# mlee03/FRE-NCtools

Hardware: AMD Instinct MI355X
Metric: exchange-cells/s (higher is better)
Workload: dtype f64; 1 GPU; C384 cubed sphere (6 tiles) -> 1440x720 lat-lon, conservative_order2: exchange-grid search + centroid pass + CSR build per step; nxgrid=4160000, parallelism=1 latitude band(s) of the target, one per GPU, world_size=1

## Files before the change

fre-nctools_amd/_lib.py:

```python
import ctypes as C
import os

_HERE = os.path.dirname(os.path.abspath(__file__))
_LIB = None


class FregridHipError(RuntimeError):
    def __init__(self, code, msg):
        super().__init__(f"libfregrid_hip error {code}: {msg}")
        self.code = code


def lib_path():
    return os.environ.get("FREGRID_HIP_LIB") or os.path.join(_HERE, "libfregrid_hip.so")


EXPORTS = [
    "get_maxxgrid", "get_grid_area", "create_xgrid_2dx2d_order1", "create_xgrid_2dx2d_order2", "conserve_interp",
    "clip_2dx2d", "poly_area", "poly_ctrlon", "poly_ctrlat", "fix_lon", "pimod",
    "fg_clip_2dx2d_batch", "fg_poly_op_batch",
    "get_maxxgrid_", "get_grid_area_", "create_xgrid_2dx2d_order1_", "create_xgrid_2dx2d_order2_",
    "fg_last_error", "fg_device_count", "fg_plan_create", "fg_plan_create_dev", "fg_plan_create_empty",
    "fg_plan_destroy", "fg_plan_set_stream", "fg_pool_release", "fg_plan_nxgrid", "fg_plan_ncells_in",
    "fg_plan_cell_sums_dev", "fg_plan_copy_cell_sums", "fg_plan_accumulate_cell_sums", "fg_plan_accumulate_cell_sums_async", "fg_dev_gather_f64", "fg_dev_scatter_f64", "fg_plan_finalize", "fg_plan_get_xgrid", "fg_plan_get_polygons", "fg_plan_create_polylist", "fg_plan_get_cell_struct",
# ... 1 lines not shown
    "fg_plan_mono_minmax_dev", "fg_plan_mono_copy_minmax", "fg_plan_mono_end",
    "fg_plan_create_great_circle", "fg_plan_create_great_circle_dev", "fg_latlon2xyz", "create_xgrid_great_circle",
    "create_xgrid_great_circle_", "get_grid_great_circle_area", "get_grid_great_circle_area_", "clip_2dx2d_great_circle",
    "great_circle_area", "fg_gc_clip_batch", "conserve_interp_great_circle", "fg_sincos_batch",
    "create_xgrid_1dx2d_order1", "create_xgrid_1dx2d_order2", "create_xgrid_2dx1d_order1", "create_xgrid_2dx1d_order2",
    "create_xgrid_1dx2d_order1_", "create_xgrid_1dx2d_order2_", "create_xgrid_2dx1d_order1_", "create_xgrid_2dx1d_order2_",
    "clip", "box_ctrlat", "box_ctrlon", "get_grid_area_no_adjust", "get_grid_area_no_adjust_", "fg_plan_stream", "fg_plan_sync",
    "fg_c2l_create", "fg_c2l_destroy", "fg_c2l_ncells", "fg_c2l_halo_size", "fg_c2l_set_stream", "fg_c2l_sync",
    "fg_c2l_get_centres", "fg_c2l_fill_halo", "fg_c2l_gradient", "fg_c2l_gradient_records", "fg_c2l_records", "fg_c2l_records_levels", "fg_c2l_grid_info", "fg_find_contacts", "fg_halo_map",
    "fg_gnomonic_ed_grid", "fg_tripolar_corners", "fg_remap_write", "fg_remap_write_interp", "fg_remap_read_size", "fg_remap_read", "fg_remap_last_error",
    "fg_plan_trim", "fg_plan_ncells_out", "fg_plan_order", "fg_plan_device", "fg_dev_alloc", "fg_dev_free", "fg_dev_upload", "fg_dev_download",
    "fg_nc_open", "fg_nc_create", "fg_nc_def_dim", "fg_nc_def_var", "fg_nc_put_att_text", "fg_nc_put_att_double", "fg_nc_enddef",
    "fg_nc_inq_ndims", "fg_nc_inq_nvars", "fg_nc_inq_numrecs", "fg_nc_inq_dimid", "fg_nc_inq_dim", "fg_nc_inq_varid", "fg_nc_inq_var",
    "fg_nc_get_att_double", "fg_nc_get_att_text", "fg_nc_get_vara", "fg_nc_get_vara_double", "fg_nc_put_vara", "fg_nc_put_vara_double",
    "fg_nc_close", "fg_nc_last_error", "fg_dev_widen", "fg_dev_narrow", "fg_sweep_create", "fg_sweep_run", "fg_sweep_run_levels", "fg_sweep_destroy", "fg_host_alloc", "fg_host_free",
    "fg_plan_stats", "fg_set_search_mode", "fg_set_search_cull", "fg_set_search_finalize", "fg_set_search_rect", "fg_set_search_wide_cap", "fg_set_search_frame", "fg_set_apply_xcd", "fg_set_apply_vec", "fg_set_apply_ep", "fg_set_gc_split", "fg_set_profiling", "fg_plan_phase_ms", "fg_gnomonic_ed_corners", "fg_latlon_corners",
    "fg_bilin_create", "fg_bilin_create_from_weights", "fg_bilin_destroy", "fg_bilin_get_index_weight", "fg_bilin_npoints_fine",
    "fg_bilin_nlon_fine", "fg_bilin_nlat_fine", "fg_bilin_nlon", "fg_bilin_nlat", "fg_bilin_ncells", "fg_bilin_set_stream",
    "fg_bilin_sync", "fg_bilin_apply_scalar", "fg_bilin_apply_vector", "fg_bilin_remap_write", "fg_bilin_remap_read",
    "fg_unit_vect_latlon", "fg_bilin_fine_grid", "fg_bilin_ambiguous_ties",
    "fg_extrap_create", "fg_extrap_destroy", "fg_extrap_set_stream", "fg_extrap_stream", "fg_extrap_run_dev", "fg_extrap_run",
    "fg_extrap_last_syncs", "fg_extrap_get_coef", "fg_extrap_coef_host", "fg_set_extrap_batch", "fg_set_extrap_coef",
    "fg_setup_vertical_interp", "fg_dev_vertical_interp",
    "fg_dev_latlon2xyz", "fg_plan_create_great_circle_lonlat", "fg_plan_create_great_circle_lonlat_dev",
    "fg_runoff_create", "fg_runoff_create_from_xgrid", "fg_runoff_destroy", "fg_runoff_nxgrid", "fg_runoff_get_xgrid",
    "fg_runoff_get_maps", "fg_runoff_get_xyz", "fg_runoff_search_stats", "fg_runoff_phase_ms", "fg_runoff_stream", "fg_runoff_apply", "fg_runoff_apply_dev",
    "fg_nearest_unmasked", "fg_set_runoff_prune", "fg_runoff_tile",
    "fg_rland_create", "fg_rland_destroy", "fg_rland_stream", "fg_rland_search", "fg_rland_search_sface", "fg_rland_stats",
    "fg_rland_phase_ms", "fg_set_rland_prune", "fg_rland_tile",
    "fg_river_create", "fg_river_destroy", "fg_river_stream", "fg_river_run", "fg_river_get", "fg_river_get_max_suba",
    "fg_river_stats", "fg_river_phase_ms", "fg_set_river_prune", "fg_river_qsort_index",
# ... 478 lines not shown
```

fre-nctools_amd/csrc/plan.hip:

```cpp
#include <hip/hip_runtime.h>
#include <math.h>
#include <stdio.h>
#include <stdlib.h>
#include <string.h>
#include <algorithm>
#include <map>
#include <mutex>
#include <string>
#include <type_traits>
#include <vector>
#include "fg_host.h"
#include "plan_internal.h"
#include "xgrid_device.h"

static thread_local std::string g_err;
extern "C" const char *fg_last_error(void) { return g_err.c_str(); }
void fg_set_last_error(const char *msg) { g_err = msg ? msg : ""; }

extern "C" int fg_device_count(void)
{
  int n = 0;
  hipError_t e = hipGetDeviceCount(&n);
  if (e != hipSuccess) { fg_fail(FG_ERR_HIP, "hipGetDeviceCount: %s", hipGetErrorString(e)); return FG_ERR_HIP; }
  return n;
}

namespace {
struct Pool {
  std::mutex mu;
  std::map<std::pair<int, size_t>, std::vector<void *>> free_;
  std::map<void *, std::pair<int, size_t>> live_;
  static size_t klass(size_t n)
  {
    size_t c = 256;
    while (c < n) c += (c < (1u << 20) ? c : (c >> 2));
    return c;
  }
  static void *poison(void *p, size_t c)
  {
    static const bool on = getenv("FREGRID_HIP_POISON") && atoi(getenv("FREGRID_HIP_POISON")) != 0;
    if (on && p) { (void)hipMemset(p, 0x7f, c); (void)hipDeviceSynchronize(); }
    return p;
  }
  void *get(int dev, size_t n) { return poison(get_raw(dev, n), klass(n ? n : 1)); }
  void *get_raw(int dev, size_t n)
  {
    if (n == 0) n = 1;
    size_t c = klass(n);
    {
      std::lock_guard<std::mutex> lk(mu);
      auto it = free_.find({dev, c});
      if (it != free_.end() && !it->second.empty()) {
        void *p = it->second.back(); it->second.pop_back();
        live_[p] = {dev, c};
        return p;
      }
    }
    void *p = nullptr;
    if (hipMalloc(&p, c) != hipSuccess) {
      release_all();
      if (hipMalloc(&p, c) != hipSuccess) return nullptr;
    }
    std::lock_guard<std::mutex> lk(mu);
    live_[p] = {dev, c};
    return p;
  }
  void put(void *p)
  {
    if (!p) return;
    std::lock_guard<std::mutex> lk(mu);
    auto it = live_.find(p);
    if (it == live_.end()) return;
    free_[it->second].push_back(p);
    live_.erase(it);
  }
  void release_all()
  {
    std::lock_guard<std::mutex> lk(mu);
    for (auto &kv : free_) for (void *p : kv.second) (void)hipFree(p);
    free_.clear();
  }
};
Pool g_pool;
}

extern "C" void fg_pool_release(void) { g_pool.release_all(); }

extern "C" void *fg_dev_alloc(size_t bytes, int device)
{
  if (hipSetDevice(device) != hipSuccess) { fg_fail(FG_ERR_HIP, "fg_dev_alloc: no such HIP device %d", device); return nullptr; }
  void *p = g_pool.get(device, bytes);
  if (!p) fg_fail(FG_ERR_HIP, "fg_dev_alloc: out of device memory (%zu bytes)", bytes);
  return p;
}
extern "C" void fg_dev_free(void *p) { g_pool.put(p); }
extern "C" int fg_dev_upload(void *dst_dev, const void *src_host, size_t bytes)
{
// ... 136 lines not shown
    }
    cv_work.notify_all();
    std::unique_lock<std::mutex> lk(mu);
    cv_done.wait(lk, [&] { return active == 0; });
    jobs = nullptr;
    return failed.load() == 0;
  }
};
XferPool &xfer_pool() { static XferPool *p = new XferPool(); return *p; }
}

static int g_profiling = 0;
extern "C" void fg_set_profiling(int on) { g_profiling = on ? 1 : 0; }
enum { PH_CELL_STRUCT = 0, PH_BINS, PH_CANDIDATES, PH_CLIP_QUAD, PH_CLIP_GENERAL, PH_COMPACT, PH_ROWS,
       PH_SEARCH_TOTAL, PH_FINALIZE, PH_APPLY, PH_COUNT };
struct HandleCache {
  std::mutex mu;
  std::map<int, std::vector<hipStream_t>> streams;
  std::map<int, std::vector<hipEvent_t>> events;
  static int current_device() { int d = 0; (void)hipGetDevice(&d); return d; }
  hipStream_t get_stream(int dev)
  {
    {
      std::lock_guard<std::mutex> lk(mu);
      auto &v = streams[dev];
      if (!v.empty()) { hipStream_t s = v.back(); v.pop_back(); return s; }
    }
    hipStream_t s = nullptr;
    if (hipStreamCreateWithFlags(&s, hipStreamNonBlocking) != hipSuccess) return nullptr;
    return s;
  }
  void put_stream(int dev, hipStream_t s)
  {
    if (!s) return;
    std::lock_guard<std::mutex> lk(mu);
    streams[dev].push_back(s);
  }
  hipEvent_t get_event()
  {
    {
      std::lock_guard<std::mutex> lk(mu);
      auto &v = events[current_device()];
      if (!v.empty()) { hipEvent_t e = v.back(); v.pop_back(); return e; }
    }
    hipEvent_t e = nullptr;
    (void)hipEventCreate(&e);
    return e;
  }
  void put_event(hipEvent_t e)
  {
    if (!e) return;
    std::lock_guard<std::mutex> lk(mu);
    events[current_device()].push_back(e);
  }
  std::map<int, std::vector<hipEvent_t>> sync_events;
  hipEvent_t get_sync_event()
  {
    {
      std::lock_guard<std::mutex> lk(mu);
      auto &v = sync_events[current_device()];
      if (!v.empty()) { hipEvent_t e = v.back(); v.pop_back(); return e; }
    }
    hipEvent_t e = nullptr;
    (void)hipEventCreateWithFlags(&e, hipEventDisableTiming);
    return e;
  }
  void put_sync_event(hipEvent_t e)
  {
    if (!e) return;
    std::lock_guard<std::mutex> lk(mu);
    sync_events[current_device()].push_back(e);
  }
};
static HandleCache g_handles;

struct PhaseTimer {
  bool on = false;
  hipStream_t st = nullptr;
  std::vector<std::pair<int, std::pair<hipEvent_t, hipEvent_t>>> spans;
  hipEvent_t open_ev = nullptr; int open_ph = -1;
  void start(bool enable, hipStream_t s) { on = enable; st = s; }
  void begin(int ph)
  {
    if (!on) return;
    open_ev = g_handles.get_event(); (void)hipEventRecord(open_ev, st); open_ph = ph;
  }
  void end()
  {
    if (!on || open_ph < 0) return;
// ... 47 lines not shown
  FgSrcRec *cen = nullptr;
  FgCsr csr{};
  int *src_idx_f = nullptr;
  double *row_sum = nullptr, *red_partial = nullptr, *red_result = nullptr;
  long row_sum_cap = 0;
  double *il_f = nullptr, *il_out = nullptr, *il_rs = nullptr;
  double *il_m = nullptr;
  unsigned char *lv_bits = nullptr;
  long stats[FG_NSTATS] = {0};
  long search_d2h = 0;
  double *mono_x = nullptr, *mono_b = nullptr;
  int *xerr = nullptr;
  bool mono_open = false;
  unsigned *ll_err = nullptr;

  template <typename T> T *alloc(size_t count)
  {
    void *p = g_pool.get(device, count * sizeof(T));
    if (p) owned.push_back(p);
    return (T *)p;
  }
  void release(void *p)
  {
    if (!p) return;
    for (size_t k = 0; k < owned.size(); k++) if (owned[k] == p) { owned.erase(owned.begin() + k); break; }
    g_pool.put(p);
  }
  void drop_search(size_t keep)
  {
    while (owned.size() > keep) { g_pool.put(owned.back()); owned.pop_back(); }
    tiles_dev = nullptr; mask_dev = nullptr; S = FgCells{}; D = FgCells{};
    x_src = x_dst = nullptr; x_area = x_c1 = x_c2 = nullptr; xoff = nullptr;
    perm = nullptr; csr.row_ptr = nullptr; csr.e1 = nullptr; csr.e2 = nullptr; cen = nullptr; src_idx_f = nullptr; sums = nullptr;
    have_geom = false; rect = false; rect_tab = FgRect{};
  }
};

static int g_wide_cap = -1;
extern "C" void fg_set_search_wide_cap(int n) { g_wide_cap = n < 0 ? -1 : n; }
static bool alloc_cells(fg_plan *pl, FgCells *c, size_t n, bool compact = false)
{
// ... 29 lines not shown
    foff += (order == 2) ? (long)(nx_in[m] + 2) * (ny_in[m] + 2) : (long)nx_in[m] * ny_in[m];
  }
  if (off > 2000000000L || (long)nx_out * ny_out > 2000000000L) { delete pl; return fg_fail(FG_ERR_ARG, "grid too large for 32-bit cell indices"); }
  pl->nsrc = (int)off; pl->f_stride = foff;
  pl->nx_out = nx_out; pl->ny_out = ny_out; pl->ndst = nx_out * ny_out;
  pl->stream = g_handles.get_stream(device);
  if (!pl->stream) { delete pl; return fg_fail(FG_ERR_HIP, "hipStreamCreate failed"); }
  *out = pl;
  return 0;
}

extern "C" void fg_plan_destroy(fg_plan *pl)
{
  if (!pl) return;
  (void)hipSetDevice(pl->device);
  if (pl->stream || !pl->own_stream) (void)hipStreamSynchronize(pl->stream);
  if (pl->stream && pl->own_stream) g_handles.put_stream(pl->device, pl->stream);
  if (pl->stream_b) { (void)hipStreamSynchronize(pl->stream_b); g_handles.put_stream(pl->device, pl->stream_b); }
  { float junk[PH_COUNT] = {0}; pl->apply_pt.collect(junk); }
  for (void *p : pl->owned) g_pool.put(p);
  delete pl;
}

static void choose_bins(const fg_plan *pl, double mean_dlat, double mean_dlon, FgBins *b)
{
  const double PI = 3.14159265358979323846;
  double h = 1.25 * mean_dlat, w = 1.25 * mean_dlon;
  int nblat = (h > 0) ? (int)ceil(PI / h) : 1;
  int nblon = (w > 0) ? (int)ceil(2.0 * PI / w) : 1;
  if (nblat < 1) nblat = 1; if (nblat > 8192) nblat = 8192;
  if (nblon < 1) nblon = 1; if (nblon > 16384) nblon = 16384;
  (void)pl;
  b->nblat = nblat; b->nblon = nblon;
  b->inv_wlat = nblat / PI;
  b->inv_wlon = nblon / (2.0 * PI);
}

static FgCounters *pinned_counters()
{
  static thread_local FgCounters *h = nullptr;
  if (!h) { if (hipHostMalloc((void **)&h, sizeof(FgCounters), hipHostMallocDefault) != hipSuccess) h = nullptr; }
  return h;
}

struct GcXyz { const double *x, *y, *z; };
struct BoxMode { FgBox box; const double *mask_quad; int no_adjust; };
struct SearchIn {
  const double *const *lon_in = nullptr, *const *lat_in = nullptr, *const *mask_in = nullptr;
  const double *lon_out = nullptr, *lat_out = nullptr;
  const GcXyz *gc_in = nullptr, *gc_out = nullptr;
  const BoxMode *boxm = nullptr;
  double mean_dlat = 0, mean_dlon = 0;
  int rect_hint = 1;
};
struct SearchOpts { bool exact, cull, finalize, rect, dst_frame; int gc_split; bool profile; };
static const char *gc_clip_error(int code)
{
  switch (code) {
    case 3: return "firstIntersect is not in the grid1List";
    case 4: return " not found the next intersection ";
    case 5: return "not return back to the first intersection";
    case 6: return "After clipping, nintersect should be 0";
    case 7: return "inserAfter: point (x,y,z) is not found in the list";
    case 8: return "Error from create_xgrid.c: temp is not in list1";
    default: return "clip_2dx2d_great_circle: more intersections than two convex quadrilaterals can have (list capacity)";
  }
}

static int g_search_cull = 0;
static int g_search_finalize = 0;
// ... 248 lines not shown
  io.dc = dc; io.xcap = nx_alloc;
  if (early_rows)
    fgd_exclusive_scan2(nacc, nsrc, pl->xoff, lb_comp, &tickets[2], &dc->xtot, row_cnt, ndst, pl->csr.row_ptr, lb_rows, &tickets[1], &dc->rows_total, dc->err, st);
  else
    fgd_exclusive_scan1(nacc, nsrc, pl->xoff, lb_comp, &tickets[2], &dc->xtot, dc->err, st);
  fgd_compact(order, nsrc, ps, io, st);
  pt.end();
  if (!early_rows) {
    pt.begin(PH_ROWS);
    fgd_exclusive_scan1(row_cnt, ndst, pl->csr.row_ptr, lb_rows, &tickets[1], &dc->rows_total, dc->err, st);
    fgd_csr_fill_pos(nx_alloc, &dc->xtot, pl->x_src, pl->x_dst, pl->csr.row_ptr, x_rowpos, pl->perm, st);
    pt.end();
  }
  ptot.end();
  const bool fuse = opt.finalize && early_rows && !pl->polys.npoly;
  int *fused_tmp = nullptr;
  if (fuse) {
    pt.begin(PH_FINALIZE);
    if (order == 2) {
      pl->cen = pl->alloc<FgSrcRec>((size_t)nsrc + 1);
      if (!pl->cen) return fg_fail(FG_ERR_HIP, "out of device memory");
      fgd_centroids(nsrc, pl->S, pl->sums, pl->cen, st);
      pl->csr.e2 = pl->alloc<FgCsrEntry2>(nx_alloc + 1);
    } else pl->csr.e1 = pl->alloc<FgCsrEntry1>(nx_alloc + 1);
    if (!pl->csr.e1 && !pl->csr.e2) return fg_fail(FG_ERR_HIP, "out of device memory");
    int *sg_tmp = pl->alloc<int>(3 * (size_t)(nx_alloc + 1));
    fgd_csr_sortgather(order, ndst, (long)nsrc + ndst, pl->perm, pl->x_area, pl->x_c1, pl->x_c2, pl->src_idx_f,
                       order == 2 ? pl->cen : nullptr, pl->csr, st, sg_tmp, nx_alloc + 1);
    fused_tmp = sg_tmp;
    pt.end();
  }
  FGCHK(hipMemcpyAsync(hc, dc, sizeof(FgCounters), hipMemcpyDeviceToHost, st));
  FGCHK(hipStreamSynchronize(st));
  pt.collect(pl->phase_ms); ptot.collect(pl->phase_ms);
  FGCHK(hipGetLastError());
  if (rect && hc->rect_bad) { caps->rect = false; return FG_RETRY; }
  if (rect && (hc->err[0] & G_ERRBIT_WIDECAP)) { caps->rect = false; return FG_RETRY; }
  if (hc->total[0] > nentries) { caps->entries = hc->total[0]; return FG_RETRY; }
  if (hc->total[0] > 2000000000ull) return fg_fail(FG_ERR_ARG, "bin table too large");
  if (hc->total[3] > (unsigned long long)ps.regcap) {
    if (hc->total[3] > 2000000000ull / (unsigned long long)ps.nreg) return fg_fail(FG_ERR_CAPACITY, "candidate pair list exceeds 2^31 entries");
    caps->regcap = (int)((hc->total[3] + FG_REG_ALIGN - 1) / FG_REG_ALIGN * FG_REG_ALIGN);
    return FG_RETRY;
  }
  if (hc->err[2] & G_ERRBIT_LL2X) return fg_fail(FG_ERR_ARG, "latlon2xyz: a grid corner is not finite, or its latitude (|lat| >= 2.4262) or longitude "
                                                          "(|lon| > 1024) lies outside the range of the device trig (radians expected)");
  if (hc->err[0] & 8u) return fg_fail(FG_ERR_ARG, "a grid corner latitude lies outside [-pi/2, pi/2] (radians expected)");
  if (hc->err[0] & 1u) return fg_fail(FG_ERR_MAXV, "create_xgrid.c: n2_in is greater than MAX_V");
// ... 5 lines not shown
  if (hc->err[0] & G_ERRBIT_GC_CLIP) return fg_fail(FG_ERR_GEOM, "%s", gc_clip_error((int)hc->err[1]));
  if (hc->err[0] & G_ERRBIT_LOOKBACK) return fg_fail(FG_ERR_HIP, "single-pass scan: a tile waited too long for its predecessor");
  pl->nx = (long)hc->xtot;
  pl->stats[FG_STAT_PAIRS] = (long)hc->total[1];
  pl->stats[FG_STAT_NONEMPTY] = (long)(hc->xtot + hc->stats[FG_STAT_BELOW]);
  pl->stats[FG_STAT_NXGRID] = pl->nx;
  pl->stats[FG_STAT_BORDERLINE] = (long)hc->stats[FG_STAT_BORDERLINE];
  pl->stats[FG_STAT_BINS] = nbins;
  pl->stats[FG_STAT_BIN_ENTRIES] = (long)hc->total[0];
  pl->stats[FG_STAT_DEFERRED] = hc->defer_cnt + hc->gc_list2_cnt;
  pl->stats[FG_STAT_HEAVY] = hc->heavy_cnt;
  pl->stats[FG_STAT_RARE] = hc->rare_cnt;
  pl->stats[FG_STAT_BELOW] = (long)hc->stats[FG_STAT_BELOW];

  pl->rect_tab.bad = nullptr;
  blk.release();
  pl->rows_built = true;
  pl->searched = true;
  if (fuse) {
    pl->release(pl->perm); pl->perm = nullptr; pl->release(fused_tmp);
    if (!pl->red_partial) { pl->red_partial = pl->alloc<double>(1024); pl->red_result = pl->alloc<double>(260); }
    if (!pl->red_partial || !pl->red_result) return fg_fail(FG_ERR_HIP, "out of device memory");
    pl->dist_pending = (order == 2);
    pl->finalized = true; pl->fused = true;
  }
  return pl->nx;
}

static int g_search_exact = 0;
extern "C" void fg_set_search_mode(int exact) { g_search_exact = exact; }
extern "C" void fg_set_search_cull(int on) { g_search_cull = on ? 1 : 0; }
extern "C" void fg_set_search_finalize(int on) { g_search_finalize = on ? 1 : 0; }
static long plan_search(fg_plan *pl, const SearchIn &in)
{
  static const bool env_exact = getenv("FREGRID_HIP_EXACT_SEARCH") && atoi(getenv("FREGRID_HIP_EXACT_SEARCH")) != 0;
  const SearchOpts opt{.exact = g_search_exact || env_exact, .cull = g_search_cull != 0, .finalize = g_search_finalize != 0,
                       .rect = g_search_rect != 0, .dst_frame = (tl_dst_frame >= 0 ? tl_dst_frame : g_dst_frame) != 0, .gc_split = g_gc_split, .profile = g_profiling != 0};
  const long big = std::max((long)pl->nsrc, (long)pl->ndst);
  if (big > (1L << 28)) return fg_fail(FG_ERR_CAPACITY, "grid of %ld cells: more than 2^28 cells per search are not supported", big);
  SearchCaps caps;
  caps.entries = opt.exact ? 0ull : 3ull * (unsigned long long)pl->ndst + 4096ull;
  const unsigned long long cap_pairs = std::min<unsigned long long>(8ull * (unsigned long long)big + 65536ull, 2000000000ull);
  caps.nreg = (int)std::max(1L, std::min((long)FG_NREG, ((long)pl->nsrc + 1023) / 1024));
  caps.regcap = opt.exact ? 0 : (int)((cap_pairs / caps.nreg + FG_REG_ALIGN - 1) / FG_REG_ALIGN * FG_REG_ALIGN);
  caps.rect = opt.rect && in.rect_hint && !in.gc_in && !in.boxm && pl->nx_out <= 8192 && pl->nx_out >= 2;
  const size_t keep = pl->owned.size();
  long rc = FG_RETRY;
  int attempts = 0;
  for (; attempts < 4 && rc == FG_RETRY; attempts++) {
    if (attempts) {
      (void)hipStreamSynchronize(pl->stream);
      pl->drop_search(keep);
    }
    rc = plan_search_core(pl, in, opt, &caps);
  }
  if (rc == FG_RETRY) return fg_fail(FG_ERR_CAPACITY, "exchange-grid search: capacities did not settle");
  if (rc >= 0) pl->stats[FG_STAT_EXACT] = (attempts > 1) ? 1 : 0;
  pl->search_d2h = (long)attempts * (long)sizeof(FgCounters);
  return rc;
}

struct CornerSample {
  int nsamp = 0;
  std::vector<double> q;
  const double *corners(int a, int k) const { return &q[((size_t)a * nsamp + k) * 4]; }
};
static long sample_step(int nx, int ny, int *nsamp)
{
  const long ncell = (long)nx * ny;
  long step = ncell / 4096; if (step < 1) step = 1;
// ... 154 lines not shown
  HostUpload &up = s->up;
  s->has_masks = mask_in != nullptr;
  for (int m = 0; m < pl->ntiles && up.ok; m++) {
    const size_t np = (size_t)(pl->nx_in[m] + 1) * (pl->ny_in[m] + 1);
    s->lon[m] = up.put(lon_in[m], np); s->lat[m] = up.put(lat_in[m], np);
    if (mask_in && mask_in[m]) s->mask[m] = up.put(mask_in[m], (size_t)pl->nx_in[m] * pl->ny_in[m]);
  }
  const size_t npo = (size_t)(pl->nx_out + 1) * (pl->ny_out + 1);
  if (up.ok) { s->lon_out = up.put(lon_out, npo); s->lat_out = up.put(lat_out, npo); }
  if (!up.run()) return fg_fail(FG_ERR_HIP, "grid upload failed (out of device memory?)");
  return 0;
}
static void adopt_stream(fg_plan *pl, void *stream)
{
  if (pl->own_stream && pl->stream) g_handles.put_stream(pl->device, pl->stream);
  pl->stream = (hipStream_t)stream; pl->own_stream = false;
}

extern "C" long fg_plan_create(int order, int ntiles_in, const int *nx_in, const int *ny_in,
                               const double *const *lon_in, const double *const *lat_in,
                               const double *const *mask_in,
                               int nx_out, int ny_out, const double *lon_out, const double *lat_out,
                               int device, fg_plan **plan_out)
{
  PlanGuard g;
  if (int rc = plan_base(order, ntiles_in, nx_in, ny_in, nx_out, ny_out, device, &g.pl)) return rc;
  StagedGrids s(g.pl);
  if (int rc = stage_host_grids(g.pl, lon_in, lat_in, mask_in, lon_out, lat_out, &s)) return rc;
  const DstExtents x = dst_extents_host(nx_out, ny_out, lon_out, lat_out);
  const long nx = plan_search(g.pl, SearchIn{.lon_in = s.lon.data(), .lat_in = s.lat.data(), .mask_in = s.masks(), .lon_out = s.lon_out,
// ... 180 lines not shown
  if (!pl->searched || !pl->have_geom) return fg_fail(FG_ERR_STATE, "fg_plan_view: needs a plan from a search");
  *v = FgPlanView{pl->nx, pl->nsrc, pl->ndst, pl->x_src, pl->x_dst, pl->x_area, pl->order == 2 ? pl->x_c1 : nullptr,
                  pl->order == 2 ? pl->x_c2 : nullptr, pl->S.area, pl->S.lon_avg};
  return 0;
}
int fg_plan_polygons_dev(const fg_plan *pl, int *n_out, double *lon, double *lat)
{
  if (!pl || !n_out || !lon || !lat) return fg_fail(FG_ERR_ARG, "null argument");
  if (!pl->searched || !pl->have_geom || !pl->x_src || pl->great_circle) return fg_fail(FG_ERR_STATE, "fg_plan_polygons_dev: needs a legacy plan from a search");
  FGCHK(hipSetDevice(pl->device));
  fgd_xgrid_polygons(pl->nx, pl->x_src, pl->x_dst, pl->S, pl->D, pl->rect ? &pl->rect_tab : nullptr, 8, n_out, lon, lat, pl->stream);
  FGCHK(hipGetLastError());
  return 0;
}
long fg_plan_search_d2h(const fg_plan *pl) { return pl ? pl->search_d2h : 0; }
void fg_dst_extents(int nx, int ny, const double *lon, const double *lat, double *dlat, double *dlon, int *rect_hint)
{
  const DstExtents x = dst_extents_host(nx, ny, lon, lat);
  *dlat = x.dlat; *dlon = x.dlon; *rect_hint = x.rect_hint;
}
int fg_search_frame_override(int frame) { const int old = tl_dst_frame; tl_dst_frame = frame; return old; }
long fg_plan_create_dev_hint(int order, int ntiles_in, const int *nx_in, const int *ny_in, const double *const *d_lon_in,
                             const double *const *d_lat_in, int nx_out, int ny_out, const double *d_lon_out, const double *d_lat_out,
                             double mean_dlat, double mean_dlon, int rect_hint, int device, void *stream, fg_plan **plan_out)
{
  PlanGuard g;
  if (int rc = plan_base(order, ntiles_in, nx_in, ny_in, nx_out, ny_out, device, &g.pl)) return rc;
  if (int rc = check_grid_ptrs(ntiles_in, {d_lon_in, d_lat_in}, {d_lon_out, d_lat_out})) return rc;
  if (!(mean_dlat > 0) || !(mean_dlon > 0)) return fg_fail(FG_ERR_ARG, "fg_plan_create_dev_hint: the extents must be positive");
  adopt_stream(g.pl, stream);
// ... 119 lines not shown
}
extern "C" void *fg_plan_stream(fg_plan *pl) { return pl ? (void *)pl->stream : nullptr; }
extern "C" int fg_plan_sync(fg_plan *pl)
{
  if (!pl) return fg_fail(FG_ERR_ARG, "null plan");
  FGCHK(hipStreamSynchronize(pl->stream));
  return 0;
}
extern "C" int fg_plan_stats(const fg_plan *pl, long *stats, int n)
{
  if (!pl || !stats) return fg_fail(FG_ERR_ARG, "null argument");
  for (int k = 0; k < n && k < FG_NSTATS; k++) stats[k] = pl->stats[k];
  return 0;
}

static int build_csr(fg_plan *pl, const FgSrcRec *cen)
{
  hipStream_t st = pl->stream;
  const int ndst = pl->ndst;
  const long nx = pl->nx;
  FGCHK(hipSetDevice(pl->device));
  if (!pl->src_idx_f) {
    pl->src_idx_f = pl->alloc<int>(pl->nsrc + 1);
    if (!pl->src_idx_f) return fg_fail(FG_ERR_HIP, "out of device memory");
    fgd_src_field_index(pl->order, pl->tiles_dev, pl->ntiles, pl->nsrc, pl->src_idx_f, st);
  }
  void *scratch = nullptr;
  if (!pl->rows_built) {
    const long t_rows = fgd_scan_tiles(ndst);
    const size_t zb = 256 + (size_t)t_rows * sizeof(unsigned long long) + 2 * ((size_t)ndst + 1) * sizeof(int);
    char *z = pl->alloc<char>(zb);
    pl->perm = pl->alloc<FgRowEnt>(nx + 1);
// ... 2 lines not shown
    FGCHK(hipMemsetAsync(z, 0, zb, st));
    unsigned long long *lb = (unsigned long long *)(z + 256);
    int *row_cnt = (int *)(z + 256 + (size_t)t_rows * sizeof(unsigned long long));
    fgd_csr_count(nx, pl->x_dst, row_cnt, st);
    fgd_exclusive_scan1(row_cnt, ndst, pl->csr.row_ptr, lb, (unsigned *)z, (unsigned long long *)(z + 8), (unsigned *)(z + 16), st);
    fgd_csr_fill(nx, pl->x_src, pl->x_dst, pl->csr.row_ptr, row_cnt + ndst + 1, pl->perm, st);
    scratch = z;
  }
  if (pl->order == 2) pl->csr.e2 = pl->alloc<FgCsrEntry2>(nx + 1);
  else pl->csr.e1 = pl->alloc<FgCsrEntry1>(nx + 1);
  if (!pl->csr.e1 && !pl->csr.e2) return fg_fail(FG_ERR_HIP, "out of device memory");
  int *sg_tmp = pl->alloc<int>(3 * (size_t)(nx + 1));
  const int long_rows = !pl->rect && !pl->great_circle && pl->stats[FG_STAT_DEFERRED] > 0 && nx > 4 * (long)ndst;
  fgd_csr_sortgather(pl->order, ndst, nx, pl->perm, pl->x_area, pl->x_c1, pl->x_c2, pl->src_idx_f, cen, pl->csr, st, sg_tmp, nx + 1,
                     long_rows);
  FGCHK(hipStreamSynchronize(st));
  FGCHK(hipGetLastError());
  pl->release(scratch); pl->release(pl->perm); pl->perm = nullptr; pl->release(sg_tmp);
  if (!pl->red_partial) { pl->red_partial = pl->alloc<double>(1024); pl->red_result = pl->alloc<double>(260); }
  if (!pl->red_partial || !pl->red_result) return fg_fail(FG_ERR_HIP, "out of device memory");
  return 0;
}

extern "C" int fg_plan_finalize(fg_plan *pl, const double *total_cell_sums_dev)
{
  if (!pl) return fg_fail(FG_ERR_ARG, "null plan");
  if (!pl->searched) return fg_fail(FG_ERR_STATE, "fg_plan_finalize: plan holds no search result");
  if (pl->finalized && pl->fused && !total_cell_sums_dev) return 0;
  if (pl->finalized) return fg_fail(FG_ERR_STATE, pl->fused ? "fg_plan_finalize: the plan was finalized by its search (fg_set_search_finalize) from its own "
                                                          "per-cell sums; totals over several plans need the two-step sequence"
                                                         : "fg_plan_finalize: already finalized");
  FGCHK(hipSetDevice(pl->device));
  PhaseTimer pt; pt.start(g_profiling != 0, pl->stream);
  pt.begin(PH_FINALIZE);
  if (pl->order == 2) {
    pl->cen = pl->alloc<FgSrcRec>((size_t)pl->nsrc + 1);
    if (!pl->cen) return fg_fail(FG_ERR_HIP, "out of device memory");
    const double *tot = total_cell_sums_dev ? total_cell_sums_dev : pl->sums;
    fgd_centroids(pl->nsrc, pl->S, tot, pl->cen, pl->stream);
    pl->dist_pending = true;
  }
  int rc = build_csr(pl, pl->order == 2 ? pl->cen : nullptr);
  if (rc) return rc;
  pt.end();
  FGCHK(hipStreamSynchronize(pl->stream));
  pl->phase_ms[PH_FINALIZE] = 0; pt.collect(pl->phase_ms);
  pl->finalized = true;
  return 0;
}

extern "C" int fg_plan_phase_ms(fg_plan *pl, float *ms, int n)
{
  if (!pl || !ms) return fg_fail(FG_ERR_ARG, "null argument");
  if (pl->apply_spans > 0) {
    FGCHK(hipSetDevice(pl->device));
    FGCHK(hipStreamSynchronize(pl->stream));
    float acc[PH_COUNT] = {0};
    pl->apply_pt.collect(acc);
    pl->phase_ms[PH_APPLY] = acc[PH_APPLY] / pl->apply_spans;
    pl->apply_spans = 0;
// ... 1250 lines not shown
```

fre-nctools_amd/csrc/plan_internal.h:

```cpp
#pragma once
#include "fregrid_hip.h"

struct FgPlanView {
  long nx;
  int nsrc, ndst;
  const int *x_src, *x_dst;
  const double *x_area, *x_c1, *x_c2;
  const double *src_area;
  const double *src_lon_avg;
};
int fg_plan_view(const fg_plan *pl, FgPlanView *v);
int fg_plan_polygons_dev(const fg_plan *pl, int *n_out, double *lon, double *lat);
long fg_plan_search_d2h(const fg_plan *pl);
void fg_dst_extents(int nx, int ny, const double *lon, const double *lat, double *dlat, double *dlon, int *rect_hint);
int fg_search_frame_override(int frame);
long fg_plan_create_dev_hint(int order, int ntiles_in, const int *nx_in, const int *ny_in, const double *const *d_lon_in,
                             const double *const *d_lat_in, int nx_out, int ny_out, const double *d_lon_out, const double *d_lat_out,
                             double mean_dlat, double mean_dlon, int rect_hint, int device, void *stream, fg_plan **plan_out);
long fg_plan_create_polylist_dev(int order, int npoly, const int *d_n, const double *d_lon, const double *d_lat, const double *d_lon_avg,
                                 const double *d_area_ref, int nx_out, int ny_out, const double *d_lon_out, const double *d_lat_out,
                                 double mean_dlat, double mean_dlon, int rect_hint, int device, void *stream, fg_plan **plan_out);
```

include/fregrid_hip.h:

```cpp
#ifndef FREGRID_HIP_H_
#define FREGRID_HIP_H_

#include <stddef.h>

#ifdef __cplusplus
extern "C" {
#endif

#define FG_ERR_ARG        (-1)
#define FG_ERR_HIP        (-2)
#define FG_ERR_MAXV       (-3)
#define FG_ERR_PARALLEL   (-4)
#define FG_ERR_CAPACITY   (-5)
#define FG_ERR_STATE      (-6)
#define FG_ERR_GEOM       (-8)
#define FG_ERR_IO         (-9)
#define FG_ERR_NOTFOUND   (-10)
#define FG_ERR_BILIN_NOTFOUND (-11)
#define FG_ERR_DATA       (-7)

#define FG_CONSERVE_ORDER1 1
#define FG_CONSERVE_ORDER2 2

int  get_maxxgrid(void);
// ... 114 lines not shown
                       const double *grad_y, const int *grad_mask);
int fg_plan_mono_minmax_dev(fg_plan *plan, double **f_min, double **f_max);
int fg_plan_mono_copy_minmax(fg_plan *plan, int to_plan, double *f_min, double *f_max);
int fg_plan_mono_end(fg_plan *plan, const fg_apply_opts *opts, const double *data, double *out, double *gsum_out);

void *fg_plan_stream(fg_plan *plan);
int fg_plan_sync(fg_plan *plan);

void fg_set_profiling(int on);
int  fg_plan_phase_ms(fg_plan *plan, float *ms, int n);

int fg_plan_stats(const fg_plan *plan, long *stats, int n);
void fg_set_search_mode(int exact);
void fg_set_search_cull(int on);
void fg_set_search_finalize(int on);
void fg_set_search_rect(int on);
void fg_set_search_wide_cap(int n);
void fg_set_search_frame(int coupler);
void fg_set_apply_ep(int on);
void fg_set_apply_vec(int v);
void fg_set_gc_split(int on);
void fg_set_apply_xcd(int on);

int fg_clip_2dx2d_batch(int npoly, const double *lon1, const double *lat1, const int *n1,
                        const double *lon2, const double *lat2, const int *n2,
                        double *lon_out, double *lat_out, int *n_out);
int fg_poly_op_batch(int op, int npoly, double *lon, double *lat, int *n, const double *clon, double *result);

typedef struct fg_c2l fg_c2l;

// ... 314 lines not shown
```

Baseline: 5.774 billion exchange-cells/s.

## Make device pool stream-ordered and drop host syncs in search/finalize

```diff
diff --git a/fre-nctools_amd/_lib.py b/fre-nctools_amd/_lib.py
--- a/fre-nctools_amd/_lib.py
+++ b/fre-nctools_amd/_lib.py
@@ -39,7 +39,7 @@
     "fg_nc_inq_ndims", "fg_nc_inq_nvars", "fg_nc_inq_numrecs", "fg_nc_inq_dimid", "fg_nc_inq_dim", "fg_nc_inq_varid", "fg_nc_inq_var",
     "fg_nc_get_att_double", "fg_nc_get_att_text", "fg_nc_get_vara", "fg_nc_get_vara_double", "fg_nc_put_vara", "fg_nc_put_vara_double",
     "fg_nc_close", "fg_nc_last_error", "fg_dev_widen", "fg_dev_narrow", "fg_sweep_create", "fg_sweep_run", "fg_sweep_run_levels", "fg_sweep_destroy", "fg_host_alloc", "fg_host_free",
-    "fg_plan_stats", "fg_set_search_mode", "fg_set_search_cull", "fg_set_search_finalize", "fg_set_search_rect", "fg_set_search_wide_cap", "fg_set_search_frame", "fg_set_apply_xcd", "fg_set_apply_vec", "fg_set_apply_ep", "fg_set_gc_split", "fg_set_profiling", "fg_plan_phase_ms", "fg_gnomonic_ed_corners", "fg_latlon_corners",
+    "fg_plan_stats", "fg_set_search_mode", "fg_set_search_cull", "fg_set_search_finalize", "fg_set_search_async", "fg_set_search_rect", "fg_set_search_wide_cap", "fg_set_search_frame", "fg_set_apply_xcd", "fg_set_apply_vec", "fg_set_apply_ep", "fg_set_gc_split", "fg_set_profiling", "fg_plan_phase_ms", "fg_gnomonic_ed_corners", "fg_latlon_corners",
     "fg_bilin_create", "fg_bilin_create_from_weights", "fg_bilin_destroy", "fg_bilin_get_index_weight", "fg_bilin_npoints_fine",
     "fg_bilin_nlon_fine", "fg_bilin_nlat_fine", "fg_bilin_nlon", "fg_bilin_nlat", "fg_bilin_ncells", "fg_bilin_set_stream",
     "fg_bilin_sync", "fg_bilin_apply_scalar", "fg_bilin_apply_vector", "fg_bilin_remap_write", "fg_bilin_remap_read",
diff --git a/fre-nctools_amd/csrc/dev_pool.h b/fre-nctools_amd/csrc/dev_pool.h
--- /dev/null
+++ b/fre-nctools_amd/csrc/dev_pool.h
@@ -0,0 +1,129 @@
+#pragma once
+#include <stddef.h>
+#include <algorithm>
+#include <map>
+#include <mutex>
+#include <utility>
+#include <vector>
+
+template <class H> struct DevPool {
+  typedef typename H::Stream Stream;
+  typedef typename H::Event Event;
+  struct Ev { Event ev; int dev; int refs; };
+  struct Batch { Ev *e; Stream stream; int dev; int refs; };
+  struct FreeBlock { void *p; Batch *batch; };
+  std::mutex mu;
+  std::map<std::pair<int, size_t>, std::vector<FreeBlock>> free_;
+  std::map<void *, std::pair<int, size_t>> live_;
+  std::vector<Batch *> open_;
+  long events_ = 0;
+
+  static size_t klass(size_t n)
+  {
+    size_t c = 256;
+    while (c < n) c += (c < (1u << 20) ? c : (c >> 2));
+    return c;
+  }
+  size_t block_bytes(void *p) { std::lock_guard<std::mutex> lk(mu); auto it = live_.find(p); return it == live_.end() ? 0 : it->second.second; }
+  long live_events() { std::lock_guard<std::mutex> lk(mu); return events_; }
+  size_t cached_blocks() { std::lock_guard<std::mutex> lk(mu); size_t n = 0; for (auto &kv : free_) n += kv.second.size(); return n; }
+
+  void *get(int dev, size_t n) { return hand_out(take(dev, n, false, Stream()), n); }
+  void *get(int dev, size_t n, Stream stream) { return hand_out(take(dev, n, true, stream), n); }
+
+  void put(void *p) { put_many(&p, 1, false, Stream(), false); }
+  void put(void *p, Stream stream, bool seal_now) { put_many(&p, 1, true, stream, seal_now); }
+  void put(const std::vector<void *> &ps, Stream stream, bool seal_now) { put_many(ps.data(), ps.size(), true, stream, seal_now); }
+
+  void seal(Stream stream) { std::lock_guard<std::mutex> lk(mu); seal_locked(stream); }
+
+  void release_all()
+  {
+    std::lock_guard<std::mutex> lk(mu);
+    for (auto &kv : free_) for (FreeBlock &b : kv.second) if (b.batch) { H::event_wait_host(event_of(b.batch)); unref(b.batch); b.batch = nullptr; }
+    for (auto &kv : free_) for (FreeBlock &b : kv.second) H::dev_free(b.p);
+    free_.clear();
+  }
+
+ private:
+  void seal_locked(Stream stream)
+  {
+    Ev *e = nullptr;
+    for (size_t k = 0; k < open_.size();) {
+      Batch *b = open_[k];
+      if (!(b->stream == stream)) { k++; continue; }
+      if (!e) { e = new Ev{H::event_get(b->dev), b->dev, 0}; events_++; H::event_record(b->dev, e->ev, stream); }
+      b->e = e; e->refs++;
+      open_.erase(open_.begin() + k);
+    }
+  }
+  Event event_of(Batch *b)
+  {
+    if (!b->e) seal_locked(b->stream);
+    return b->e->ev;
+  }
+  void unref(Batch *b)
+  {
+    if (--b->refs > 0) return;
+    if (b->e) { if (--b->e->refs == 0) { H::event_put(b->e->dev, b->e->ev); events_--; delete b->e; } }
+    else open_.erase(std::find(open_.begin(), open_.end(), b));
+    delete b;
+  }
+  void *hand_out(void *p, size_t n)
+  {
+    if (p && H::poison_on()) H::poison(p, klass(n ? n : 1));
+    return p;
+  }
+  void *take(int dev, size_t n, bool on_stream, Stream stream)
+  {
+    if (n == 0) n = 1;
+    const size_t c = klass(n);
+    {
+      std::lock_guard<std::mutex> lk(mu);
+      auto it = free_.find({dev, c});
+      if (it != free_.end() && !it->second.empty()) {
+        std::vector<FreeBlock> &v = it->second;
+        int best = -1, best_rank = 4;
+        for (int k = (int)v.size() - 1; k >= 0 && best_rank > 0; k--) {
+          const Batch *b = v[k].batch;
+          const int rank = (!b || (on_stream && b->stream == stream)) ? 0 : 3;
+          if (rank < best_rank || (rank == 3 && best_rank == 3)) { best = k; best_rank = rank; }
+        }
+        if (best_rank == 3)
+          for (int k = (int)v.size() - 1; k >= 0; k--)
+            if (v[k].batch->e && H::event_passed(v[k].batch->e->ev)) { best = k; best_rank = 2; break; }
+        FreeBlock fb = v[best];
+        v.erase(v.begin() + best);
+        if (fb.batch) {
+          if (best_rank == 3) { if (on_stream) H::stream_wait(stream, event_of(fb.batch)); else H::event_wait_host(event_of(fb.batch)); }
+          unref(fb.batch);
+        }
+        live_[fb.p] = {dev, c};
+        return fb.p;
+      }
+    }
+    void *p = H::dev_malloc(c);
+    if (!p) {
+      release_all();
+      p = H::dev_malloc(c);
+      if (!p) return nullptr;
+    }
+    std::lock_guard<std::mutex> lk(mu);
+    live_[p] = {dev, c};
+    return p;
+  }
+  void put_many(void *const *ps, size_t n, bool tagged, Stream stream, bool seal_now)
+  {
+    std::lock_guard<std::mutex> lk(mu);
+    Batch *b = nullptr;
+    for (size_t k = 0; k < n; k++) {
+      auto it = live_.find(ps[k]);
+      if (!ps[k] || it == live_.end()) continue;
+      if (tagged && !b) { b = new Batch{nullptr, stream, it->second.first, 0}; open_.push_back(b); }
+      if (b) b->refs++;
+      free_[it->second].push_back(FreeBlock{ps[k], b});
+      live_.erase(it);
+    }
+    if (tagged && seal_now) seal_locked(stream);
+  }
+};
diff --git a/fre-nctools_amd/csrc/plan.hip b/fre-nctools_amd/csrc/plan.hip
--- a/fre-nctools_amd/csrc/plan.hip
+++ b/fre-nctools_amd/csrc/plan.hip
@@ -25,62 +25,96 @@
   return n;
 }
 
+struct HandleCache {
+  std::mutex mu;
+  std::map<int, std::vector<hipStream_t>> streams;
+  std::map<int, std::vector<hipEvent_t>> events;
+  static int current_device() { int d = 0; (void)hipGetDevice(&d); return d; }
+  hipStream_t get_stream(int dev)
+  {
+    {
+      std::lock_guard<std::mutex> lk(mu);
+      auto &v = streams[dev];
+      if (!v.empty()) { hipStream_t s = v.back(); v.pop_back(); return s; }
+    }
+    hipStream_t s = nullptr;
+    if (hipStreamCreateWithFlags(&s, hipStreamNonBlocking) != hipSuccess) return nullptr;
+    return s;
+  }
+  void put_stream(int dev, hipStream_t s)
+  {
+    if (!s) return;
+    std::lock_guard<std::mutex> lk(mu);
+    streams[dev].push_back(s);
+  }
+  hipEvent_t get_event()
+  {
+    {
+      std::lock_guard<std::mutex> lk(mu);
+      auto &v = events[current_device()];
+      if (!v.empty()) { hipEvent_t e = v.back(); v.pop_back(); return e; }
+    }
+    hipEvent_t e = nullptr;
+    (void)hipEventCreate(&e);
+    return e;
+  }
+  void put_event(hipEvent_t e)
+  {
+    if (!e) return;
+    std::lock_guard<std::mutex> lk(mu);
+    events[current_device()].push_back(e);
+  }
+  std::map<int, std::vector<hipEvent_t>> sync_events;
+  hipEvent_t get_sync_event(int dev = -1)
+  {
+    {
+      std::lock_guard<std::mutex> lk(mu);
+      auto &v = sync_events[dev >= 0 ? dev : current_device()];
+      if (!v.empty()) { hipEvent_t e = v.back(); v.pop_back(); return e; }
+    }
+    hipEvent_t e = nullptr;
+    if (hipEventCreateWithFlags(&e, hipEventDisableTiming) != hipSuccess) { (void)hipGetLastError(); return nullptr; }
+    return e;
+  }
+  void put_sync_event(hipEvent_t e, int dev = -1)
+  {
+    if (!e) return;
+    std::lock_guard<std::mutex> lk(mu);
+    sync_events[dev >= 0 ? dev : current_device()].push_back(e);
+  }
+};
+static HandleCache g_handles;
+
+#include "dev_pool.h"
 namespace {
-struct Pool {
-  std::mutex mu;
-  std::map<std::pair<int, size_t>, std::vector<void *>> free_;
-  std::map<void *, std::pair<int, size_t>> live_;
-  static size_t klass(size_t n)
+struct HipPoolPolicy {
+  typedef hipStream_t Stream;
+  typedef hipEvent_t Event;
+  static void *dev_malloc(size_t c) { void *p = nullptr; if (hipMalloc(&p, c) != hipSuccess) { (void)hipGetLastError(); return nullptr; } return p; }
+  static void dev_free(void *p) { (void)hipFree(p); }
+  struct OnDevice {
+    int old = -1, dev;
+    explicit OnDevice(int d) : dev(d) { if (hipGetDevice(&old) != hipSuccess) old = -1; if (old != dev) (void)hipSetDevice(dev); }
+    ~OnDevice() { if (old >= 0 && old != dev) (void)hipSetDevice(old); }
+  };
+  static Event event_get(int dev) { OnDevice on(dev); return g_handles.get_sync_event(dev); }
+  static void event_put(int dev, Event e) { g_handles.put_sync_event(e, dev); }
+  static void event_record(int dev, Event e, Stream s)
   {
-    size_t c = 256;
-    while (c < n) c += (c < (1u << 20) ? c : (c >> 2));
-    return c;
-  }
-  static void *poison(void *p, size_t c)
+    OnDevice on(dev);
+    if (!e || hipEventRecord(e, s) != hipSuccess) { (void)hipGetLastError(); (void)hipDeviceSynchronize(); }
+  }
+  static bool event_passed(Event e) { return !e || hipEventQuery(e) != hipErrorNotReady; }
+  static void stream_wait(Stream s, Event e) { if (e && hipStreamWaitEvent(s, e, 0) != hipSuccess) (void)hipEventSynchronize(e); }
+  static void event_wait_host(Event e) { if (e) (void)hipEventSynchronize(e); }
+  static bool poison_on()
   {
     static const bool on = getenv("FREGRID_HIP_POISON") && atoi(getenv("FREGRID_HIP_POISON")) != 0;
-    if (on && p) { (void)hipMemset(p, 0x7f, c); (void)hipDeviceSynchronize(); }
-    return p;
-  }
-  void *get(int dev, size_t n) { return poison(get_raw(dev, n), klass(n ? n : 1)); }
-  void *get_raw(int dev, size_t n)
-  {
-    if (n == 0) n = 1;
-    size_t c = klass(n);
-    {
-      std::lock_guard<std::mutex> lk(mu);
-      auto it = free_.find({dev, c});
-      if (it != free_.end() && !it->second.empty()) {
-        void *p = it->second.back(); it->second.pop_back();
-        live_[p] = {dev, c};
-        return p;
-      }
-    }
-    void *p = nullptr;
-    if (hipMalloc(&p, c) != hipSuccess) {
-      release_all();
-      if (hipMalloc(&p, c) != hipSuccess) return nullptr;
-    }
-    std::lock_guard<std::mutex> lk(mu);
-    live_[p] = {dev, c};
-    return p;
-  }
-  void put(void *p)
-  {
-    if (!p) return;
-    std::lock_guard<std::mutex> lk(mu);
-    auto it = live_.find(p);
-    if (it == live_.end()) return;
-    free_[it->second].push_back(p);
-    live_.erase(it);
-  }
-  void release_all()
-  {
-    std::lock_guard<std::mutex> lk(mu);
-    for (auto &kv : free_) for (void *p : kv.second) (void)hipFree(p);
-    free_.clear();
-  }
+    return on;
+  }
+  static void poison(void *p, size_t c) { (void)hipDeviceSynchronize(); (void)hipMemset(p, 0x7f, c); (void)hipDeviceSynchronize(); }
 };
+typedef DevPool<HipPoolPolicy> Pool;
 Pool g_pool;
 }
 
@@ -247,65 +281,6 @@
 extern "C" void fg_set_profiling(int on) { g_profiling = on ? 1 : 0; }
 enum { PH_CELL_STRUCT = 0, PH_BINS, PH_CANDIDATES, PH_CLIP_QUAD, PH_CLIP_GENERAL, PH_COMPACT, PH_ROWS,
        PH_SEARCH_TOTAL, PH_FINALIZE, PH_APPLY, PH_COUNT };
-struct HandleCache {
-  std::mutex mu;
-  std::map<int, std::vector<hipStream_t>> streams;
-  std::map<int, std::vector<hipEvent_t>> events;
-  static int current_device() { int d = 0; (void)hipGetDevice(&d); return d; }
-  hipStream_t get_stream(int dev)
-  {
-    {
-      std::lock_guard<std::mutex> lk(mu);
-      auto &v = streams[dev];
-      if (!v.empty()) { hipStream_t s = v.back(); v.pop_back(); return s; }
-    }
-    hipStream_t s = nullptr;
-    if (hipStreamCreateWithFlags(&s, hipStreamNonBlocking) != hipSuccess) return nullptr;
-    return s;
-  }
-  void put_stream(int dev, hipStream_t s)
-  {
-    if (!s) return;
-    std::lock_guard<std::mutex> lk(mu);
-    streams[dev].push_back(s);
-  }
-  hipEvent_t get_event()
-  {
-    {
-      std::lock_guard<std::mutex> lk(mu);
-      auto &v = events[current_device()];
-      if (!v.empty()) { hipEvent_t e = v.back(); v.pop_back(); return e; }
-    }
-    hipEvent_t e = nullptr;
-    (void)hipEventCreate(&e);
-    return e;
-  }
-  void put_event(hipEvent_t e)
-  {
-    if (!e) return;
-    std::lock_guard<std::mutex> lk(mu);
-    events[current_device()].push_back(e);
-  }
-  std::map<int, std::vector<hipEvent_t>> sync_events;
-  hipEvent_t get_sync_event()
-  {
-    {
-      std::lock_guard<std::mutex> lk(mu);
-      auto &v = sync_events[current_device()];
-      if (!v.empty()) { hipEvent_t e = v.back(); v.pop_back(); return e; }
-    }
-    hipEvent_t e = nullptr;
-    (void)hipEventCreateWithFlags(&e, hipEventDisableTiming);
-    return e;
-  }
-  void put_sync_event(hipEvent_t e)
-  {
-    if (!e) return;
-    std::lock_guard<std::mutex> lk(mu);
-    sync_events[current_device()].push_back(e);
-  }
-};
-static HandleCache g_handles;
 
 struct PhaseTimer {
   bool on = false;
@@ -383,17 +358,25 @@
   bool mono_open = false;
   unsigned *ll_err = nullptr;
 
+  bool async = false, on_stream = false;
+
   template <typename T> T *alloc(size_t count)
   {
-    void *p = g_pool.get(device, count * sizeof(T));
+    void *p = on_stream ? g_pool.get(device, count * sizeof(T), stream) : g_pool.get(device, count * sizeof(T));
     if (p) owned.push_back(p);
     return (T *)p;
   }
+  void disown(void *p) { for (size_t k = 0; k < owned.size(); k++) if (owned[k] == p) { owned.erase(owned.begin() + k); break; } }
   void release(void *p)
   {
     if (!p) return;
-    for (size_t k = 0; k < owned.size(); k++) if (owned[k] == p) { owned.erase(owned.begin() + k); break; }
+    disown(p);
     g_pool.put(p);
+  }
+  void release_on_stream(const std::vector<void *> &ps)
+  {
+    for (void *p : ps) disown(p);
+    g_pool.put(ps, stream, false);
   }
   void drop_search(size_t keep)
   {
@@ -453,11 +436,13 @@
 {
   if (!pl) return;
   (void)hipSetDevice(pl->device);
-  if (pl->stream || !pl->own_stream) (void)hipStreamSynchronize(pl->stream);
+  const bool drain = !pl->async || !pl->apply_pt.spans.empty();
+  if (drain && (pl->stream || !pl->own_stream)) (void)hipStreamSynchronize(pl->stream);
+  if (pl->stream_b) { if (drain) (void)hipStreamSynchronize(pl->stream_b); g_handles.put_stream(pl->device, pl->stream_b); }
+  { float junk[PH_COUNT] = {0}; pl->apply_pt.collect(junk); }
+  if (pl->async) g_pool.put(pl->owned, pl->stream, !pl->own_stream);
+  else for (void *p : pl->owned) g_pool.put(p);
   if (pl->stream && pl->own_stream) g_handles.put_stream(pl->device, pl->stream);
-  if (pl->stream_b) { (void)hipStreamSynchronize(pl->stream_b); g_handles.put_stream(pl->device, pl->stream_b); }
-  { float junk[PH_COUNT] = {0}; pl->apply_pt.collect(junk); }
-  for (void *p : pl->owned) g_pool.put(p);
   delete pl;
 }
 
@@ -475,11 +460,12 @@
   b->inv_wlon = nblon / (2.0 * PI);
 }
 
+struct PinnedCounters { FgCounters c; unsigned long long mark; };
 static FgCounters *pinned_counters()
 {
-  static thread_local FgCounters *h = nullptr;
-  if (!h) { if (hipHostMalloc((void **)&h, sizeof(FgCounters), hipHostMallocDefault) != hipSuccess) h = nullptr; }
-  return h;
+  static thread_local PinnedCounters *h = nullptr;
+  if (!h) { if (hipHostMalloc((void **)&h, sizeof(PinnedCounters), hipHostMallocCoherent) != hipSuccess) h = nullptr; else h->mark = 0; }
+  return h ? &h->c : nullptr;
 }
 
 struct GcXyz { const double *x, *y, *z; };
@@ -492,7 +478,29 @@
   double mean_dlat = 0, mean_dlon = 0;
   int rect_hint = 1;
 };
-struct SearchOpts { bool exact, cull, finalize, rect, dst_frame; int gc_split; bool profile; };
+struct SearchOpts { bool exact, cull, finalize, rect, dst_frame; int gc_split; bool profile, async; };
+__global__ __launch_bounds__(64) void k_counters_out(const unsigned *src, unsigned *dst, int nwords, unsigned long long *mark, unsigned long long seq)
+{
+  for (int k = threadIdx.x; k < nwords; k += 64) dst[k] = src[k];
+  __threadfence_system();
+  __syncthreads();
+  if (threadIdx.x == 0) __hip_atomic_store(mark, seq, __ATOMIC_RELEASE, __HIP_MEMORY_SCOPE_SYSTEM);
+}
+static_assert(sizeof(FgCounters) % sizeof(unsigned) == 0 && offsetof(PinnedCounters, mark) == sizeof(FgCounters), "FgCounters travels as 32-bit words, the mark behind them");
+static hipError_t wait_counters(const FgCounters *hc, unsigned long long seq, hipStream_t st)
+{
+  const unsigned long long *mark = &((const PinnedCounters *)hc)->mark;
+  for (unsigned spin = 1;; spin++) {
+    if (__atomic_load_n(mark, __ATOMIC_ACQUIRE) == seq) return hipSuccess;
+    __builtin_ia32_pause();
+    if (spin % 65536 == 0) {
+      const hipError_t e = hipStreamQuery(st);
+      if (e == hipErrorNotReady) (void)hipGetLastError();
+      if (e == hipSuccess) return __atomic_load_n(mark, __ATOMIC_ACQUIRE) == seq ? hipSuccess : hipErrorUnknown;
+      if (e != hipErrorNotReady) return e;
+    }
+  }
+}
 static const char *gc_clip_error(int code)
 {
   switch (code) {
@@ -771,24 +779,39 @@
   }
   ptot.end();
   const bool fuse = opt.finalize && early_rows && !pl->polys.npoly;
+  const bool stream_ordered = fuse && opt.async && !opt.profile;
+  static thread_local unsigned long long rb_seq = 0;
   int *fused_tmp = nullptr;
   if (fuse) {
+    if (order == 2) { pl->cen = pl->alloc<FgSrcRec>((size_t)nsrc + 1); pl->csr.e2 = pl->alloc<FgCsrEntry2>(nx_alloc + 1); }
+    else pl->csr.e1 = pl->alloc<FgCsrEntry1>(nx_alloc + 1);
+    if ((order == 2 && !pl->cen) || (!pl->csr.e1 && !pl->csr.e2)) return fg_fail(FG_ERR_HIP, "out of device memory");
+    fused_tmp = pl->alloc<int>(3 * (size_t)(nx_alloc + 1));
+  }
+  if (stream_ordered) {
+    unsigned *hc_dev = nullptr;
+    if (hipHostGetDevicePointer((void **)&hc_dev, hc, 0) != hipSuccess || !hc_dev) return fg_fail(FG_ERR_HIP, "the counters' host block is not mapped");
+    const int nwords = (int)(sizeof(FgCounters) / sizeof(unsigned));
+    k_counters_out<<<1, 64, 0, st>>>((const unsigned *)dc, hc_dev, nwords, (unsigned long long *)(hc_dev + nwords), ++rb_seq);
+    FGCHK(hipGetLastError());
+  }
+  if (fuse) {
     pt.begin(PH_FINALIZE);
-    if (order == 2) {
-      pl->cen = pl->alloc<FgSrcRec>((size_t)nsrc + 1);
-      if (!pl->cen) return fg_fail(FG_ERR_HIP, "out of device memory");
-      fgd_centroids(nsrc, pl->S, pl->sums, pl->cen, st);
-      pl->csr.e2 = pl->alloc<FgCsrEntry2>(nx_alloc + 1);
-    } else pl->csr.e1 = pl->alloc<FgCsrEntry1>(nx_alloc + 1);
-    if (!pl->csr.e1 && !pl->csr.e2) return fg_fail(FG_ERR_HIP, "out of device memory");
-    int *sg_tmp = pl->alloc<int>(3 * (size_t)(nx_alloc + 1));
+    if (order == 2) fgd_centroids(nsrc, pl->S, pl->sums, pl->cen, st);
     fgd_csr_sortgather(order, ndst, (long)nsrc + ndst, pl->perm, pl->x_area, pl->x_c1, pl->x_c2, pl->src_idx_f,
-                       order == 2 ? pl->cen : nullptr, pl->csr, st, sg_tmp, nx_alloc + 1);
-    fused_tmp = sg_tmp;
+                       order == 2 ? pl->cen : nullptr, pl->csr, st, fused_tmp, nx_alloc + 1);
     pt.end();
   }
-  FGCHK(hipMemcpyAsync(hc, dc, sizeof(FgCounters), hipMemcpyDeviceToHost, st));
-  FGCHK(hipStreamSynchronize(st));
+  if (stream_ordered) {
+    if (hipError_t e = hipGetLastError()) {
+      (void)hipStreamSynchronize(st);
+      return fg_fail(FG_ERR_HIP, "a launch of the search failed: %s", hipGetErrorString(e));
+    }
+    FGCHK(wait_counters(hc, rb_seq, st));
+  } else {
+    FGCHK(hipMemcpyAsync(hc, dc, sizeof(FgCounters), hipMemcpyDeviceToHost, st));
+    FGCHK(hipStreamSynchronize(st));
+  }
   pt.collect(pl->phase_ms); ptot.collect(pl->phase_ms);
   FGCHK(hipGetLastError());
   if (rect && hc->rect_bad) { caps->rect = false; return FG_RETRY; }
@@ -824,6 +847,11 @@
   pl->stats[FG_STAT_BELOW] = (long)hc->stats[FG_STAT_BELOW];
 
   pl->rect_tab.bad = nullptr;
+  if (stream_ordered) {
+    blk.scratch.push_back(pl->perm); blk.scratch.push_back(fused_tmp);
+    pl->release_on_stream(blk.scratch); blk.scratch.clear();
+    pl->perm = nullptr; fused_tmp = nullptr;
+  }
   blk.release();
   pl->rows_built = true;
   pl->searched = true;
@@ -841,11 +869,13 @@
 extern "C" void fg_set_search_mode(int exact) { g_search_exact = exact; }
 extern "C" void fg_set_search_cull(int on) { g_search_cull = on ? 1 : 0; }
 extern "C" void fg_set_search_finalize(int on) { g_search_finalize = on ? 1 : 0; }
+static int g_search_async = 1;
+extern "C" void fg_set_search_async(int on) { g_search_async = on ? 1 : 0; }
 static long plan_search(fg_plan *pl, const SearchIn &in)
 {
   static const bool env_exact = getenv("FREGRID_HIP_EXACT_SEARCH") && atoi(getenv("FREGRID_HIP_EXACT_SEARCH")) != 0;
   const SearchOpts opt{.exact = g_search_exact || env_exact, .cull = g_search_cull != 0, .finalize = g_search_finalize != 0,
-                       .rect = g_search_rect != 0, .dst_frame = (tl_dst_frame >= 0 ? tl_dst_frame : g_dst_frame) != 0, .gc_split = g_gc_split, .profile = g_profiling != 0};
+                       .rect = g_search_rect != 0, .dst_frame = (tl_dst_frame >= 0 ? tl_dst_frame : g_dst_frame) != 0, .gc_split = g_gc_split, .profile = g_profiling != 0, .async = g_search_async != 0};
   const long big = std::max((long)pl->nsrc, (long)pl->ndst);
   if (big > (1L << 28)) return fg_fail(FG_ERR_CAPACITY, "grid of %ld cells: more than 2^28 cells per search are not supported", big);
   SearchCaps caps;
@@ -857,6 +887,8 @@
   const size_t keep = pl->owned.size();
   long rc = FG_RETRY;
   int attempts = 0;
+  pl->async = opt.async;
+  pl->on_stream = pl->async;
   for (; attempts < 4 && rc == FG_RETRY; attempts++) {
     if (attempts) {
       (void)hipStreamSynchronize(pl->stream);
@@ -864,6 +896,7 @@
     }
     rc = plan_search_core(pl, in, opt, &caps);
   }
+  pl->on_stream = false;
   if (rc == FG_RETRY) return fg_fail(FG_ERR_CAPACITY, "exchange-grid search: capacities did not settle");
   if (rc >= 0) pl->stats[FG_STAT_EXACT] = (attempts > 1) ? 1 : 0;
   pl->search_d2h = (long)attempts * (long)sizeof(FgCounters);
@@ -1048,6 +1081,7 @@
 static void adopt_stream(fg_plan *pl, void *stream)
 {
   if (pl->own_stream && pl->stream) g_handles.put_stream(pl->device, pl->stream);
+  else if (!pl->own_stream) g_pool.seal(pl->stream);
   pl->stream = (hipStream_t)stream; pl->own_stream = false;
 }
 
@@ -1258,6 +1292,13 @@
   return 0;
 }
 long fg_plan_search_d2h(const fg_plan *pl) { return pl ? pl->search_d2h : 0; }
+extern "C" long fg_plan_device_bytes(const fg_plan *pl, long *sizes, int nmax)
+{
+  if (!pl) return 0;
+  long sum = 0;
+  for (size_t k = 0; k < pl->owned.size(); k++) { const long b = (long)g_pool.block_bytes(pl->owned[k]); sum += b; if (sizes && (int)k < nmax) sizes[k] = b; }
+  return sum;
+}
 void fg_dst_extents(int nx, int ny, const double *lon, const double *lat, double *dlat, double *dlon, int *rect_hint)
 {
   const DstExtents x = dst_extents_host(nx, ny, lon, lat);
@@ -1407,8 +1448,14 @@
   return 0;
 }
 
+static bool finalize_stream_ordered(const fg_plan *pl) { return pl->async && !pl->own_stream && !g_profiling; }
 static int build_csr(fg_plan *pl, const FgSrcRec *cen)
 {
+  struct OnStream {
+    fg_plan *pl; bool was;
+    ~OnStream() { pl->on_stream = was; }
+  } on_stream{pl, pl->on_stream};
+  pl->on_stream = pl->async;
   hipStream_t st = pl->stream;
   const int ndst = pl->ndst;
   const long nx = pl->nx;
@@ -1441,9 +1488,14 @@
   const int long_rows = !pl->rect && !pl->great_circle && pl->stats[FG_STAT_DEFERRED] > 0 && nx > 4 * (long)ndst;
   fgd_csr_sortgather(pl->order, ndst, nx, pl->perm, pl->x_area, pl->x_c1, pl->x_c2, pl->src_idx_f, cen, pl->csr, st, sg_tmp, nx + 1,
                      long_rows);
-  FGCHK(hipStreamSynchronize(st));
+  if (finalize_stream_ordered(pl)) {
+    pl->release_on_stream({scratch, pl->perm, sg_tmp});
+  } else {
+    FGCHK(hipStreamSynchronize(st));
+    pl->release(scratch); pl->release(pl->perm); pl->release(sg_tmp);
+  }
+  pl->perm = nullptr;
   FGCHK(hipGetLastError());
-  pl->release(scratch); pl->release(pl->perm); pl->perm = nullptr; pl->release(sg_tmp);
   if (!pl->red_partial) { pl->red_partial = pl->alloc<double>(1024); pl->red_result = pl->alloc<double>(260); }
   if (!pl->red_partial || !pl->red_result) return fg_fail(FG_ERR_HIP, "out of device memory");
   return 0;
@@ -1461,7 +1513,9 @@
   PhaseTimer pt; pt.start(g_profiling != 0, pl->stream);
   pt.begin(PH_FINALIZE);
   if (pl->order == 2) {
+    pl->on_stream = pl->async;
     pl->cen = pl->alloc<FgSrcRec>((size_t)pl->nsrc + 1);
+    pl->on_stream = false;
     if (!pl->cen) return fg_fail(FG_ERR_HIP, "out of device memory");
     const double *tot = total_cell_sums_dev ? total_cell_sums_dev : pl->sums;
     fgd_centroids(pl->nsrc, pl->S, tot, pl->cen, pl->stream);
@@ -1470,7 +1524,7 @@
   int rc = build_csr(pl, pl->order == 2 ? pl->cen : nullptr);
   if (rc) return rc;
   pt.end();
-  FGCHK(hipStreamSynchronize(pl->stream));
+  if (!finalize_stream_ordered(pl)) FGCHK(hipStreamSynchronize(pl->stream));
   pl->phase_ms[PH_FINALIZE] = 0; pt.collect(pl->phase_ms);
   pl->finalized = true;
   return 0;
diff --git a/fre-nctools_amd/csrc/plan_internal.h b/fre-nctools_amd/csrc/plan_internal.h
--- a/fre-nctools_amd/csrc/plan_internal.h
+++ b/fre-nctools_amd/csrc/plan_internal.h
@@ -12,6 +12,7 @@
 int fg_plan_view(const fg_plan *pl, FgPlanView *v);
 int fg_plan_polygons_dev(const fg_plan *pl, int *n_out, double *lon, double *lat);
 long fg_plan_search_d2h(const fg_plan *pl);
+extern "C" long fg_plan_device_bytes(const fg_plan *pl, long *sizes, int nmax);
 void fg_dst_extents(int nx, int ny, const double *lon, const double *lat, double *dlat, double *dlon, int *rect_hint);
 int fg_search_frame_override(int frame);
 long fg_plan_create_dev_hint(int order, int ntiles_in, const int *nx_in, const int *ny_in, const double *const *d_lon_in,
diff --git a/include/fregrid_hip.h b/include/fregrid_hip.h
--- a/include/fregrid_hip.h
+++ b/include/fregrid_hip.h
@@ -152,6 +152,7 @@
 void fg_set_search_mode(int exact);
 void fg_set_search_cull(int on);
 void fg_set_search_finalize(int on);
+void fg_set_search_async(int on);
 void fg_set_search_rect(int on);
 void fg_set_search_wide_cap(int n);
 void fg_set_search_frame(int coupler);
```

After: 5.962 billion exchange-cells/s (median of 6 runs). +3.2%, better.
